# ylongqi/openrec

Hardware: AMD Instinct MI355X
Metric: BPR training triplets/sec at dim=64, 1Mx1M table (higher is better)
Workload: dtype f32; 1 GPU; bpr dim=64 1000000x1000000 table, batch=65536 triplets/GPU, sgd lr=0.05, objective loss+l2_loss, exact TF duplicate semantics; parallelism=single-gpu

## Files before the change

### include/openrec_hip.h

```cpp
#ifndef OPENREC_HIP_H
#define OPENREC_HIP_H

#include <stdint.h>

#ifdef __cplusplus
extern "C" {
#endif

typedef struct orx_ctx orx_ctx;
typedef struct orx_table orx_table;
typedef struct orx_opt orx_opt;

enum orx_status {
    ORX_OK = 0,
    ORX_ERR_ARG = -1,
    ORX_ERR_HIP = -2,
    ORX_ERR_OOM = -3,
    ORX_ERR_INDEX = -4,
    ORX_ERR_STATE = -5
};

enum orx_opt_kind { ORX_SGD = 0, ORX_ADAGRAD = 1, ORX_ADAM = 2, ORX_MOMENTUM = 3 };

enum orx_pair_model { ORX_BPR = 0, ORX_UCML = 1 };
// ... 262 lines not shown
int orx_prof_get(orx_ctx* ctx, int kid, double* total_ms, int64_t* launches);
int orx_ctx_stat(orx_ctx* ctx, int what, int64_t* out);
int orx_copy_bandwidth(orx_ctx* ctx, int64_t bytes, int32_t reps, double* gbps_out);

int orx_gemm16_plan(int32_t num_cu, int32_t M, int32_t N, int32_t K, int64_t lda, int64_t ldb, int32_t* nt_out, int32_t* tn_out);
int orx_gemm16_group_query(int32_t num_cu, int32_t B, int32_t in, int32_t out, int64_t ldx, int64_t lddz, int64_t ldw, int32_t nt_cols,
                           int32_t* plan_out);
int orx_gemm16_nt(orx_ctx* ctx, const void* A16, int64_t lda, const void* B16, int64_t ldb, float* C, int64_t ldc, void* C16, int64_t ldc16,
                  const float* bias, int32_t M, int32_t N, int32_t K, int act, const float* actY, const void* actY16, int64_t ldy, int act_y,
                  float* colparts, int32_t* P_out, void* mask_out, const void* mask_in);
int orx_gemm16_tn(orx_ctx* ctx, const void* A16, int64_t lda, const void* B16, int64_t ldb, float* C, int64_t ldc, float* slab,
                  int32_t M, int32_t N, int32_t K, float out_scale);
int orx_gemm16_group(orx_ctx* ctx, const void* X16, int64_t ldx, const void* dZ16, int64_t lddz, float* gW, int64_t ldgw, float* slab,
                     int32_t in, int32_t out, int32_t B, float out_scale, const void* W16, int64_t ldw, float* C, int64_t ldc,
                     void* C16, int64_t ldc16, const float* actY, const void* actY16, int64_t ldy, int act_y, float* colparts,
                     int32_t* P_out, const void* mask_in, int32_t nt_cols);
int orx_head16_fwd(orx_ctx* ctx, const void* X16, int64_t ldx, const void* w16, const float* bias, int act, float* pred, int32_t B, int32_t K);
int32_t orx_head16_bwd_blocks(orx_ctx* ctx, int32_t B);
int orx_head16_bwd(orx_ctx* ctx, const void* X16, int64_t ldx, const void* w16, const float* dy, const float* pred, int act, int act_below,
                   float* gW_parts, float* gb_parts, void* dZ16, int64_t ld16, float* dZ32, int64_t ld32, float* gb_below_parts,
                   int32_t B, int32_t K, int32_t* P_out);
int orx_cast16(orx_ctx* ctx, const float* src, int64_t lds, void* dst16, int64_t ld16, int32_t M, int32_t N);

int orx_plan_geometry(int64_t NU, int64_t NI, int64_t nU, int64_t nP, int64_t nN, int32_t* out);
int orx_plan_dump(orx_ctx* ctx, const int32_t* uid, const int32_t* pid, const int32_t* nid, const float* label, int64_t K, int64_t B,
                  int64_t NU, int64_t NI, int32_t D, const int32_t* opts, void* const* out, int64_t* info);

#ifdef __cplusplus
}
#endif
#endif
```

### openrec_amd/_ffi.py

```python
from __future__ import annotations

import ctypes
import os
from ctypes import POINTER, c_char_p, c_double, c_float, c_int, c_int32, c_int64, c_size_t, c_uint64, c_void_p

HERE = os.path.dirname(os.path.abspath(__file__))
LIB_PATH = os.environ.get("ORX_LIB_PATH") or os.path.join(HERE, "_lib", "libopenrec_hip.so")

ORX_OK, ORX_ERR_ARG, ORX_ERR_HIP, ORX_ERR_OOM, ORX_ERR_INDEX, ORX_ERR_STATE = 0, -1, -2, -3, -4, -5
ORX_SGD, ORX_ADAGRAD, ORX_ADAM, ORX_MOMENTUM = 0, 1, 2, 3
ORX_BPR, ORX_UCML = 0, 1
ORX_GMF, ORX_WRMF = 0, 1
ORX_IDS_DEVICE, ORX_HOGWILD, ORX_NO_L2, ORX_CENSOR, ORX_POINT_SIGMOID, ORX_OUT_DEVICE = 1, 2, 4, 8, 16, 32
ORX_TRAIN_USER, ORX_TRAIN_ITEM, ORX_TRAIN_BIAS = 1, 2, 4
ORX_SHARD_OVERLAP, ORX_SHARD_NO_DEDUP, ORX_SHARD_DEDUP, ORX_COMM_ID_BYTES = 0x100, 0x200, 0x400, 128
ORX_DLRM_INTERACT_ITSELF, ORX_DLRM_SIGMOID_BOT, ORX_DLRM_SIGMOID_TOP, ORX_DLRM_LOSS_BCE, ORX_DLRM_REFERENCE_COMPAT = 1, 2, 4, 8, 16
ORX_DLRM_FP16_MLP = 32
ORX_DLRM_NO_EMB = 64
ORX_K_DEDUP, ORX_K_FUSED, ORX_K_REDUCE, ORX_K_SWEEP, ORX_K_CENSOR, ORX_K_POINT, ORX_K_DUPAPPLY, ORX_K_GEMM, ORX_K_NUM = 0, 1, 2, 3, 4, 5, 6, 7, 8
KERNEL_NAMES = {ORX_K_DEDUP: "dedup", ORX_K_FUSED: "fused", ORX_K_REDUCE: "loss_reduce", ORX_K_SWEEP: "adam_sweep",
                ORX_K_CENSOR: "censor", ORX_K_POINT: "pointwise", ORX_K_DUPAPPLY: "dup_apply", ORX_K_GEMM: "gemm"}

_p = c_void_p
_pp = POINTER(c_void_p)
# ... 102 lines not shown
    "orx_shard_grads_sgd": (c_int, [_p, c_int, _p, _p, _fp, _ip, _ip, _p, _p, _p, _ip, _fp, _p, c_int64, c_int64, c_int64, c_float, c_int, _fp, _ip, _fp, _p]),
    "orx_shard_request_dedup_steps": (c_int, [_p, _ip, c_int64, c_int64, c_int32, c_int32, c_int64, _ip, _ip, _ip, _p, _p, _p, _ip, _ip]),
    "orx_prof_enable": (c_int, [_p, c_int]),
    "orx_prof_reset": (c_int, [_p]),
    "orx_prof_get": (c_int, [_p, c_int, POINTER(c_double), POINTER(c_int64)]),
    "orx_ctx_stat": (c_int, [_p, c_int, POINTER(c_int64)]),
    "orx_copy_bandwidth": (c_int, [_p, c_int64, c_int32, POINTER(c_double)]),
    "orx_mlp_forward": (c_int, [_p, c_int32, POINTER(_p), POINTER(_p), POINTER(c_int32), _p, c_int64, c_int32, c_int, _p]),
    "orx_interact_forward": (c_int, [_p, _p, c_int64, c_int32, c_int32, c_int, c_int, c_int, _p]),
    "orx_gemm16_plan": (c_int, [c_int32, c_int32, c_int32, c_int32, c_int64, c_int64, POINTER(c_int32), POINTER(c_int32)]),
    "orx_gemm16_group_query": (c_int, [c_int32, c_int32, c_int32, c_int32, c_int64, c_int64, c_int64, c_int32, POINTER(c_int32)]),
    "orx_gemm16_nt": (c_int, [_p, _p, c_int64, _p, c_int64, _fp, c_int64, _p, c_int64, _fp, c_int32, c_int32, c_int32, c_int,
                              _fp, _p, c_int64, c_int, _fp, POINTER(c_int32), _p, _p]),
    "orx_gemm16_tn": (c_int, [_p, _p, c_int64, _p, c_int64, _fp, c_int64, _fp, c_int32, c_int32, c_int32, c_float]),
    "orx_gemm16_group": (c_int, [_p, _p, c_int64, _p, c_int64, _fp, c_int64, _fp, c_int32, c_int32, c_int32, c_float, _p, c_int64, _fp, c_int64,
                                 _p, c_int64, _fp, _p, c_int64, c_int, _fp, POINTER(c_int32), _p, c_int32]),
    "orx_head16_fwd": (c_int, [_p, _p, c_int64, _p, _fp, c_int, _fp, c_int32, c_int32]),
    "orx_head16_bwd_blocks": (c_int32, [_p, c_int32]),
    "orx_head16_bwd": (c_int, [_p, _p, c_int64, _p, _fp, _fp, c_int, c_int, _fp, _fp, _p, c_int64, _fp, c_int64, _fp, c_int32, c_int32, POINTER(c_int32)]),
    "orx_cast16": (c_int, [_p, _fp, c_int64, _p, c_int64, c_int32, c_int32]),
    "orx_plan_geometry": (c_int, [c_int64, c_int64, c_int64, c_int64, c_int64, POINTER(c_int32)]),
    "orx_plan_dump": (c_int, [_p, _ip, _ip, _ip, _fp, c_int64, c_int64, c_int64, c_int64, c_int32, POINTER(c_int32), POINTER(c_void_p),
                              POINTER(c_int64)]),
}

_lib = None


class OrxError(RuntimeError):
    def __init__(self, code, msg):
        super().__init__(f"[orx {code}] {msg}")
        self.code = code


def load():
    global _lib
    if _lib is not None:
        return _lib
    if not os.path.exists(LIB_PATH):
        raise ImportError(
            f"{LIB_PATH} is missing: build it with `python -m openrec_amd.build` "
            "(hipcc, gfx950).  openrec_amd has no CPU fallback.")
    try:
        import torch
    except ImportError:
        pass
# ... 21 lines not shown
```

### openrec_amd/csrc/api_plan.hip

```cpp
#include "orx_internal.h"

#include <cstring>
#include <vector>

#define CHECK(call)                                                                    \
    do {                                                                               \
        int _rc = (call);                                                              \
        if (_rc != ORX_OK) return _rc;                                                 \
    } while (0)

extern "C" int orx_plan_geometry(int64_t NU, int64_t NI, int64_t nU, int64_t nP, int64_t nN, int32_t* out) {
    ORX_ARG(out && NU > 0 && NI > 0 && nU >= 0 && nP >= 0 && nN >= 0, "orx_plan_geometry: bad argument");
    DedupArgs d;
    memset(&d, 0, sizeof(d));
    d.nU = nU; d.nP = nP; d.nN = nN; d.NU = NU; d.NI = NI;
    orx_plan_geometry_query(d, out);
    out[14] = (int32_t)orx_dedup_range_rows(); out[15] = orx_dedup_buckets(NU);
    return ORX_OK;
}

namespace {
struct DevBuf {
    void* p = nullptr;
    ~DevBuf() { if (p) (void)hipFree(p); }
    int put(const void* src, size_t bytes, hipStream_t st) {
        ORX_HIP(hipMalloc(&p, bytes < 16 ? 16 : bytes));
        ORX_HIP(hipMemcpyAsync(p, src, bytes, hipMemcpyHostToDevice, st));
        return ORX_OK;
    }
};
template <class T>
int fetch(std::vector<T>* h, const T* dev, size_t n, hipStream_t st) {
    h->resize(n);
    if (n) ORX_HIP(hipMemcpyAsync(h->data(), dev, n * sizeof(T), hipMemcpyDeviceToHost, st));
    return ORX_OK;
}
}

extern "C" int orx_plan_dump(orx_ctx* c, const int32_t* uid, const int32_t* pid, const int32_t* nid, const float* label, int64_t K, int64_t B,
                             int64_t NU, int64_t NI, int32_t D, const int32_t* opts, void* const* out, int64_t* info) {
// ... 116 lines not shown
```

### openrec_amd/csrc/kernels_plan.hip

```cpp
#include "orx_internal.h"

#include "orx_device.h"

#include <cstring>
#include <vector>
#include <algorithm>

constexpr int PL_THREADS = 256;
constexpr int PL_REFS = 8;
constexpr int PL_CHUNK = PL_THREADS * PL_REFS;
constexpr int PL_LCNT = 1024;

struct PlanArgs {
    DedupArgs d;
    int shift;
    int nru, nri;
    int lgu, lgi;
    int* bcnt;
    int2* list;
    int64_t nref;
    unsigned int* dupbits;
    int min_late;
    int s_first;
    unsigned long long* tstamp;
};
#define PL_STAMP(i) do { if (a.tstamp != nullptr && threadIdx.x == 0) a.tstamp[((size_t)blockIdx.y * gridDim.x + blockIdx.x) * 8 + (i)] = wall_clock64(); } while (0)

__device__ __forceinline__ bool plan_ref(const PlanArgs& a, int64_t s, int64_t j, int& id, bool& is_user, int& pos) {
    const DedupArgs& d = a.d;
    if (j < d.nU) { id = d.uid[s * d.id_stride + j]; is_user = true; pos = (int)j; }
    else if (j < d.nU + d.nP) { id = d.pid[s * d.id_stride + (j - d.nU)]; is_user = false; pos = (int)(d.role_stride ? d.role_stride + (j - d.nU) : j); }
    else { id = d.nid[s * d.id_stride + (j - d.nU - d.nP)]; is_user = false; pos = (int)(d.role_stride ? 2 * d.role_stride + (j - d.nU - d.nP) : j); }
    return id_ok(id, is_user ? d.NU : d.NI);
}

__device__ __forceinline__ int32_t* plan_idword(const DedupArgs& d, int64_t s, int pos) {
    if (d.pair_tpw > 1) {
        const int Bp = (int)d.role_stride;
        const int slot = (pos >= Bp ? 1 : 0) + (pos >= 2 * Bp ? 1 : 0);
        return reinterpret_cast<int32_t*>(d.ids4 + s * d.pair_stride + (pos - slot * Bp)) + slot;
    }
    return d.ids_out + s * d.flag_stride + pos;
}

__device__ __forceinline__ void pl_lds_barrier() { asm volatile("s_waitcnt lgkmcnt(0)\n\ts_barrier" ::: "memory"); }

template <int T = PL_THREADS>
__device__ __forceinline__ int plan_scan_excl(int v, int* wave_tot, int& total) {
    const int lane = threadIdx.x & 63, wave = threadIdx.x >> 6;
    int incl = v;
#pragma unroll
    for (int o = 1; o < 64; o <<= 1) { const int t = __shfl_up(incl, o); if (lane >= o) incl += t; }
    if (lane == 63) wave_tot[wave] = incl;
    pl_lds_barrier();
    int before = 0, all = 0;
#pragma unroll
    for (int k = 0; k < T / 64; ++k) { const int t = wave_tot[k]; if (k < wave) before += t; all += t; }
    pl_lds_barrier();
    total = all;
    return before + incl - v;
}

template <bool SCATTER>
__global__ __launch_bounds__(PL_THREADS) void plan_part_kernel(PlanArgs a) {
    extern __shared__ int pl_hist[];
    const int nb = a.nru + a.nri;
    const int64_t s = blockIdx.y;
    int* hist = pl_hist;
    int* base = pl_hist + nb;
    for (int i = threadIdx.x; i < nb; i += PL_THREADS) hist[i] = 0;
    __syncthreads();
    const int64_t j0 = (int64_t)blockIdx.x * PL_CHUNK + threadIdx.x;
    int bk[PL_REFS], rk[PL_REFS], idv[PL_REFS], posv[PL_REFS];
#pragma unroll
    for (int k = 0; k < PL_REFS; ++k) {
        const int64_t j = j0 + (int64_t)k * PL_THREADS;
        bk[k] = -1;
        if (j < a.nref) {
            int id, pos; bool is_user;
            const bool ok = plan_ref(a, s, j, id, is_user, pos);
            if (ok) {
                bk[k] = is_user ? (id & (a.nru - 1)) : a.nru + (id & (a.nri - 1));
                idv[k] = id; posv[k] = pos;
            }
            if (SCATTER) {
                if (a.d.pair_tpw > 1) {
                    if (j < a.d.pair_stride) {
                        const int p = a.d.pid[s * a.d.id_stride + j];
                        const int n = a.d.label ? __float_as_int(a.d.label[s * a.d.id_stride + j]) : a.d.nid[s * a.d.id_stride + j];
                        const bool okp = id_ok(p, a.d.NI), okn = a.d.label ? true : id_ok(n, a.d.NI);
                        a.d.ids4[s * a.d.pair_stride + j] = make_int4(ok ? id : 0x7fffffff, okp ? p : 0x7fffffff, okn ? n : 0x7fffffff, (int)((uint32_t)j << 10));
                        if (!(ok & okp & okn)) {
                            const int poison = (int)(ORX_PARTNER_POISON | ((uint32_t)a.d.pair_gen << 24));
                            a.d.partner[s * a.d.pair_stride + j] = make_int4(poison, poison, poison, 0);
                        }
                    }
                } else {
                    a.d.ids_out[s * a.d.flag_stride + pos] = ok ? id : 0x7fffffff;
                }
            }
        }
    }
#pragma unroll
    for (int k = 0; k < PL_REFS; ++k) if (bk[k] >= 0) rk[k] = atomicAdd(&hist[bk[k]], 1);
    __syncthreads();
    int* cnt = a.bcnt + s * (3 * nb + 1);
    if (!SCATTER) {
        if (blockIdx.x == 0 && threadIdx.x < 8) a.d.alloc[8 * s + threadIdx.x] = 0;
        if (blockIdx.x == 0 && threadIdx.x == 8) a.d.dcount[s] = 0;
        for (int i = threadIdx.x; i < nb; i += PL_THREADS) { const int c = hist[i]; if (c) atomicAdd(cnt + i, c); }
        return;
    }
    __shared__ int wave_tot[PL_THREADS / 64];
    int* off = pl_hist + 2 * nb;
    for (int i = threadIdx.x; i < nb; i += PL_THREADS) off[i] = cnt[i];
    __syncthreads();
    {
        const int per = (nb + PL_THREADS - 1) / PL_THREADS;
        const int i0 = threadIdx.x * per;
        int mine = 0;
        for (int i = i0; i < i0 + per && i < nb; ++i) mine += off[i];
        int total;
        int run = plan_scan_excl(mine, wave_tot, total);
        for (int i = i0; i < i0 + per && i < nb; ++i) { const int c = off[i]; off[i] = run; run += c; }
        if (threadIdx.x == 0) off[nb] = total;
    }
    __syncthreads();
    if (blockIdx.x == 0) for (int i = threadIdx.x; i <= nb; i += PL_THREADS) cnt[2 * nb + i] = off[i];
    int* cur = cnt + nb;
    for (int i = threadIdx.x; i < nb; i += PL_THREADS) { const int c = hist[i]; if (c) base[i] = off[i] + atomicAdd(cur + i, c); }
    __syncthreads();
    int2* list = a.list + s * a.nref;
#pragma unroll
    for (int k = 0; k < PL_REFS; ++k) if (bk[k] >= 0) list[base[bk[k]] + rk[k]] = make_int2(idv[k], posv[k]);
}

__device__ __forceinline__ int pl_cnt(const int* p) { return __hip_atomic_load(p, __ATOMIC_RELAXED, __HIP_MEMORY_SCOPE_AGENT); }
__device__ __forceinline__ unsigned int pl_peek(const unsigned int* p) { return *reinterpret_cast<const volatile unsigned int*>(p); }

constexpr int PL_UN = 8;
template <int T, class F>
__device__ __forceinline__ void pl_for_each(const int2* ent, int n, F f) {
    for (int i0 = threadIdx.x; i0 < n; i0 += PL_UN * T) {
        int2 e[PL_UN];
#pragma unroll
        for (int k = 0; k < PL_UN; ++k) { const int i = i0 + k * T; if (i < n) e[k] = ent[i]; }
#pragma unroll
        for (int k = 0; k < PL_UN; ++k) { const int i = i0 + k * T; if (i < n) f(i, e[k]); }
    }
}

__device__ __forceinline__ int pl_rank(int* cnt, int dn) {
    const int lane = threadIdx.x & 63;
    int rank = -1;
    for (int round = 0; round < 4; ++round) {
        const unsigned long long todo = __ballot(rank < 0);
        if (!todo) break;
        const int ld = __shfl(dn, __ffsll((long long)todo) - 1);
        const bool mine = rank < 0 && dn == ld;
        const unsigned long long grp = __ballot(mine);
        const int gsz = __popcll(grp);
        if (gsz < 4) break;
        const int first = __ffsll((long long)grp) - 1;
        int base = 0;
        if (lane == first) base = atomicAdd(cnt + ld, gsz);
        base = __shfl(base, first);
        if (mine) rank = base + __popcll(grp & ((1ull << lane) - 1ull));
    }
    if (rank < 0) rank = atomicAdd(cnt + dn, 1);
    return rank;
}

constexpr int PL_PAIR_CAP = 512;

template <int T>
__global__ __launch_bounds__(T) void plan_range_kernel(PlanArgs a) {
    extern __shared__ __attribute__((aligned(16))) unsigned int pl_lds[];
    const DedupArgs& d = a.d;
    const int W = (1 << a.shift) >> 5;
    unsigned int* seen = pl_lds;
    unsigned int* dup = pl_lds + W;
    unsigned int* tri = pl_lds + 2 * W;
    unsigned short* prefix16 = reinterpret_cast<unsigned short*>(pl_lds + 3 * W);
    int* lcnt = reinterpret_cast<int*>(pl_lds + 3 * W + (W + 1) / 2);
    unsigned short* dprefix16 = reinterpret_cast<unsigned short*>(seen);
    int* pairpos = reinterpret_cast<int*>(lcnt + PL_LCNT);
    __shared__ int wave_tot[T / 64];
    __shared__ int sh_late, sh_dense, sh_seg, list_cnt, list_base;
    const int nb = a.nru + a.nri;
    const int b = blockIdx.x;
    const int64_t s = blockIdx.y;
    const bool is_user = b < a.nru;
    const int lg = is_user ? a.lgu : a.lgi;
    const int bl = is_user ? b : b - a.nru;
    const int* cnt = a.bcnt + s * (3 * nb + 1) + 2 * nb;
    PL_STAMP(0);
    if (b == 0) for (int i = threadIdx.x; i < 2 * nb; i += T) a.bcnt[s * (3 * nb + 1) + i] = 0;
    const int lo = cnt[b], n = cnt[b + 1] - lo;
    int2* ent = a.list + s * a.nref + lo;
    unsigned int* dupout = a.dupbits ? a.dupbits + ((size_t)s * nb + b) * W : nullptr;
    if (threadIdx.x == 0 && n > 8192) atomicMax(d.alloc + 8 * s + 6, n);
    if (n == 0) {
        if (dupout) for (int w = threadIdx.x; w < W; w += T) dupout[w] = 0u;
        return;
    }
    int2* refinfo = d.refinfo ? d.refinfo + s * d.flag_stride : nullptr;
    const bool small = n <= PL_UN * T;
    int2 er[PL_UN];
    if (small) {
// ... 42 lines not shown
    int off = 0;
    if (mine) off = atomicAdd(&list_cnt, mine);
    pl_lds_barrier();
    int list_base_r = 0;
    if (threadIdx.x == 0 && list_cnt) {
        list_base_r = atomicAdd(d.dcount + s, list_cnt);
        atomicAdd(d.alloc + 8 * s + 5, list_cnt);
    }
    const bool want_plan = sh_late >= (a.min_late < 0 ? (n / 512 > 64 ? n / 512 : 64) : a.min_late);
    const bool plan = refinfo != nullptr && want_plan;
    if (want_plan && refinfo == nullptr && threadIdx.x == 0) atomicAdd(d.alloc + 8 * s + 1, sh_late);
    int ntri = 0, dense0 = 0;
    int* segstart = nullptr;
    if (plan) {
        segstart = d.segstart + s * d.tri_stride;
        const int per = (W + T - 1) / T;
        const int w0 = threadIdx.x * per;
        int mine3 = 0;
        for (int w = w0; w < w0 + per && w < W; ++w) mine3 += __popc(tri[w]);
        int pre = plan_scan_excl<T>(mine3, wave_tot, ntri);
        if (ntri > 65535) ntri = 0;
        if (ntri) {
            if (threadIdx.x == 0) sh_dense = atomicAdd(d.alloc + 8 * s, ntri);
            for (int w = w0; w < w0 + per && w < W; ++w) { prefix16[w] = (unsigned short)pre; pre += __popc(tri[w]); }
            __syncthreads();
            dense0 = sh_dense;
            if (ntri > PL_LCNT) lcnt = d.tricnt + s * d.tri_stride + dense0;
            for (int i = threadIdx.x; i < ntri; i += T) lcnt[i] = 0;
            __syncthreads();
        }
    }
    int ndup2 = 0;
    const bool pairing = d.pair_tpw > 1 && W <= 4096;
    if (pairing) {
        const int per = (W + T - 1) / T;
        const int w0 = threadIdx.x * per;
        int mine2 = 0;
        for (int w = w0; w < w0 + per && w < W; ++w) mine2 += __popc(dup[w] & ~tri[w]);
        int pre = plan_scan_excl<T>(mine2, wave_tot, ndup2);
        if (ndup2 > PL_PAIR_CAP) ndup2 = 0;
        if (ndup2) {
            for (int w = w0; w < w0 + per && w < W; ++w) { dprefix16[w] = (unsigned short)pre; pre += __popc(dup[w] & ~tri[w]); }
            for (int i = threadIdx.x; i < 2 * ndup2; i += T) pairpos[i] = -1;
            pl_lds_barrier();
        }
    }
    PL_STAMP(3);
    auto pass2 = [&](int2 e) {
        const int l = e.x >> lg;
        const int pos = e.y & 0x3fffffff;
        const unsigned int dw = dup[l >> 5];
        const unsigned int dd = (dw >> (l & 31)) & 1u;
        if (dd) {
            uint32_t v = (uint32_t)e.x | (1u << 31);
            const unsigned int tw = tri[l >> 5];
            const unsigned int t3 = (tw >> (l & 31)) & 1u;
            if (ndup2 && !t3) {
                const int dn2 = (int)dprefix16[l >> 5] + __popc(dw & ~tw & ((1u << (l & 31)) - 1u));
                pairpos[2 * dn2 + (int)(((uint32_t)e.y >> 30) & 1u)] = pos;
                return;
            }
            v |= (t3 ? 2u : ((uint32_t)e.y >> 30)) << 29;
            if (t3 && ntri) {
                const int dn = (int)prefix16[l >> 5] + __popc(tw & ((1u << (l & 31)) - 1u));
                refinfo[pos] = make_int2(dense0 + dn, pl_rank(lcnt, dn));
            } else if (t3 && refinfo != nullptr) {
                refinfo[pos] = make_int2(-1, 0);
            }
            *plan_idword(d, s, pos) = (int32_t)v;
        }
    };
    if (small) {
#pragma unroll
        for (int k = 0; k < PL_UN; ++k) { const int i = threadIdx.x + k * T; if (i < n) pass2(er[k]); }
    } else {
        pl_for_each<T>(ent, n, [&](int, int2 e) { pass2(e); });
    }
    PL_STAMP(4);
    if (ndup2) {
        pl_lds_barrier();
        int* partner = reinterpret_cast<int*>(d.partner + s * d.pair_stride);
        const int Bp = (int)d.role_stride;
        for (int k = threadIdx.x; k < ndup2; k += T) {
            const int posA = pairpos[2 * k], posB = pairpos[2 * k + 1];
            const int sa = (posA >= Bp ? 1 : 0) + (posA >= 2 * Bp ? 1 : 0), sb = (posB >= Bp ? 1 : 0) + (posB >= 2 * Bp ? 1 : 0);
            const int tag = d.pair_gen << 24;
            partner[4 * (posA - sa * Bp) + sa] = posB | tag;
// ... 22 lines not shown
    PL_STAMP(7);
    if (mine) {
        int64_t e = s * d.list_stride + list_base + off;
        const uint32_t tag = is_user ? 0u : 0x80000000u;
        for (int w = threadIdx.x; w < W; w += T) {
            unsigned int m = dup[w];
            const unsigned int m0 = m;
            const unsigned int tw = tri[w];
            while (m) {
                const int bpos = __ffs(m) - 1;
                m &= m - 1;
                if (ndup2 && !((tw >> bpos) & 1u)) {
                    const int dn2 = (int)dprefix16[w] + __popc(m0 & ~tw & ((1u << bpos) - 1u));
                    reinterpret_cast<int2*>(d.pslot)[e] = make_int2(pairpos[2 * dn2], pairpos[2 * dn2 + 1]);
                    if (d.dcnt != nullptr) { d.dseg[e] = 0; d.dcnt[e] = 0; }
                    ++e;
                    continue;
                }
                if (d.pair_tpw > 1) reinterpret_cast<int2*>(d.pslot)[e] = make_int2(-1, -1);
                d.dlist[e] = (uint32_t)((((int64_t)w * 32 + bpos) << lg) | bl) | tag;
                if (d.dcnt != nullptr) {
                    int c = 0, sg = 0;
                    if (ntri && ((tw >> bpos) & 1u)) {
                        const int dn = (int)prefix16[w] + __popc(tw & ((1u << bpos) - 1u));
                        c = pl_cnt(lcnt + dn);
                        sg = __hip_atomic_load(segstart + dense0 + dn, __ATOMIC_RELAXED, __HIP_MEMORY_SCOPE_AGENT);
                        if (c > ORX_SEG_DIRECT) {
                            int4* items = d.items + s * d.item_stride;
                            int src = sg, len = c, level = 0;
                            do {
                                const int pieces = (len + ORX_PIECE - 1) / ORX_PIECE;
                                const int b0 = d.tree_off[level] + atomicAdd(d.alloc + 8 * s + 2 + level, pieces);
                                for (int k = 0; k < pieces; ++k) {
                                    const int rem = len - k * ORX_PIECE;
                                    items[b0 + k] = make_int4(src + k * ORX_PIECE, rem < ORX_PIECE ? rem : ORX_PIECE, b0 + k, 0);
                                }
                                src = b0; len = pieces; ++level;
                            } while (len > ORX_SEG_DIRECT && level < 3);
                            sg = src; c = -len;
                        }
                    }
                    d.dseg[e] = sg; d.dcnt[e] = c;
                }
                ++e;
            }
        }
    }
// ... 92 lines not shown
        }
    }
    __shared__ int sh_np;
    if (threadIdx.x == 0) sh_np = 0;
    __syncthreads();
    if (npair) atomicAdd(&sh_np, npair);
    __syncthreads();
    if (threadIdx.x == 0 && sh_np) atomicAdd(d.alloc + 8 * s + 7, sh_np);
}

__global__ __launch_bounds__(256) void plan_swap_kernel(DedupArgs d) {
    const int64_t s = blockIdx.y;
    const int n = d.dcount[s];
    int4* rec = d.ids4 + s * d.pair_stride;
    for (int e = blockIdx.x * 256 + threadIdx.x; e < n; e += gridDim.x * 256) {
        const int2 qm = reinterpret_cast<const int2*>(d.pslot)[s * d.list_stride + e];
        if (qm.x < 0 || qm.y < 0) continue;
        const int4 a = rec[qm.x], b = rec[qm.y];
        rec[qm.x] = make_int4(b.x, b.y, b.z, a.w);
        rec[qm.y] = make_int4(a.x, a.y, a.z, b.w);
    }
}

int orx_launch_plan_swap(orx_ctx* ctx, const DedupArgs& d, int64_t kc) {
    if (d.pair_tpw < 2 || kc <= 0) return ORX_OK;
    ProfScope ps(ctx, ORX_K_DEDUP);
    ORX_LAUNCH(ctx, plan_swap_kernel, dim3((unsigned)std::max<int64_t>(4, (d.pair_stride / 4 + 255) / 256), (unsigned)kc), dim3(256), 0, d);
    ORX_HIP(hipGetLastError());
    return ORX_OK;
}

static int plan_buckets(int64_t rows, int64_t nref_t) {
    if (rows <= 0 || nref_t <= 0) return 0;
    const int cap = rows > (1LL << 27) ? 18 : 17;
    int64_t want = std::max<int64_t>((rows + (1LL << cap) - 1) >> cap, std::min<int64_t>(nref_t / 2048, rows / 64));
    static const char* env = getenv("ORX_PLAN_SHIFT");
    if (env) want = std::max<int64_t>(want, (rows + (1LL << atoi(env)) - 1) >> atoi(env));
    int n = 1;
    while (n < want && n < 8192) n *= 2;
    return n;
}
static int ilog2(int64_t n) { int l = 0; while ((1LL << l) < n) ++l; return l; }
static void plan_geometry(const DedupArgs& d, PlanArgs* a) {
    a->nref = d.nU + d.nP + d.nN;
    a->nru = plan_buckets(d.nU ? d.NU : 0, d.nU);
    a->nri = plan_buckets((d.nP + d.nN) ? d.NI : 0, d.nP + d.nN);
    a->lgu = ilog2(a->nru > 0 ? a->nru : 1); a->lgi = ilog2(a->nri > 0 ? a->nri : 1);
    const int64_t per_u = a->nru ? (d.NU + a->nru - 1) / a->nru : 1, per_i = a->nri ? (d.NI + a->nri - 1) / a->nri : 1;
    a->shift = std::max(5, ilog2(std::max(per_u, per_i)));
}

void orx_plan_geometry_query(const DedupArgs& d, int32_t out[14]) {
    PlanArgs a;
    plan_geometry(d, &a);
    out[0] = a.nru; out[1] = a.nri; out[2] = a.lgu; out[3] = a.lgi; out[4] = a.shift; out[5] = (1 << a.shift) >> 5;
    out[6] = PL_UN; out[7] = PL_LCNT; out[8] = PL_PAIR_CAP; out[9] = ORX_SEG_DIRECT; out[10] = ORX_PIECE;
    out[11] = PL_THREADS; out[12] = 1024; out[13] = PL_CHUNK;
}

static int plan_ensure(orx_ctx* c, int64_t chunk, const PlanArgs& a, bool want_dupbits) {
    const int nb = a.nru + a.nri;
    if (orx_ensure((void**)&c->d_pl_cnt, &c->d_pl_cnt_cap, (size_t)chunk * (3 * nb + 1) * sizeof(int))) return ORX_ERR_OOM;
    if (orx_ensure((void**)&c->d_pl_list, &c->d_pl_list_cap, (size_t)chunk * a.nref * sizeof(int2))) return ORX_ERR_OOM;
    const size_t words = (size_t)nb * ((1u << a.shift) >> 5);
    if (want_dupbits && orx_ensure((void**)&c->d_dupbits, &c->d_dupbits_cap, (size_t)chunk * words * sizeof(unsigned int))) return ORX_ERR_OOM;
    return ORX_OK;
}

int orx_plan_buffers(orx_ctx* c, int64_t chunk, int64_t B, int64_t NU, int64_t NI, bool want_dupbits) {
    const int64_t shapes[3][3] = {{B, B, B}, {B, B, 0}, {0, B, 0}};
    for (const auto& sh : shapes) {
        DedupArgs d;
        memset(&d, 0, sizeof(d));
        d.nU = sh[0]; d.nP = sh[1]; d.nN = sh[2]; d.NU = NU; d.NI = NI;
        PlanArgs a;
        plan_geometry(d, &a);
        const int rc = plan_ensure(c, chunk, a, want_dupbits);
        if (rc != ORX_OK) return rc;
    }
    return ORX_OK;
// ... 5 lines not shown
    a.d = d;
    plan_geometry(d, &a);
    const int nb = a.nru + a.nri;
    if (nb == 0 || a.nref == 0 || kc == 0) return ORX_OK;
    ORX_ARG(a.nref < (1LL << 30) && kc < 65536, "plan: too many references per step (%lld) or steps (%lld)", (long long)a.nref, (long long)kc);
    { const int rc = plan_ensure(ctx, step0 + kc, a, keep_dupbits); if (rc != ORX_OK) return rc; }
    const size_t words = (size_t)nb * ((1u << a.shift) >> 5);
    a.bcnt = ctx->d_pl_cnt + step0 * (3 * nb + 1); a.list = ctx->d_pl_list + step0 * a.nref;
    a.dupbits = keep_dupbits ? ctx->d_dupbits + step0 * words : nullptr;
    a.s_first = 1;
    a.tstamp = nullptr;
    static const bool timing = getenv("ORX_PLAN_TIMING") != nullptr;
    if (timing) {
        ORX_HIP(hipMalloc((void**)&a.tstamp, (size_t)nb * kc * 8 * sizeof(unsigned long long)));
        ORX_HIP(hipMemsetAsync(a.tstamp, 0, (size_t)nb * kc * 8 * sizeof(unsigned long long), ctx->stream));
    }
    const char* ml = getenv("ORX_PLAN_MIN_LATE");
    a.min_late = ml ? atoi(ml) : d.min_late;
    if (ctx->pl_cnt_clean != ctx->d_pl_cnt || ctx->pl_cnt_clean_cap != ctx->d_pl_cnt_cap || ctx->pl_cnt_nb != nb)
        ORX_HIP(hipMemsetAsync(ctx->d_pl_cnt, 0, ctx->d_pl_cnt_cap, ctx->stream));
    ctx->pl_cnt_clean = nullptr;
    struct CleanMark { orx_ctx* c; int nb; bool ok = false;
                       ~CleanMark() { if (ok) { c->pl_cnt_clean = c->d_pl_cnt; c->pl_cnt_clean_cap = c->d_pl_cnt_cap; c->pl_cnt_nb = nb; } } } clean_mark{ctx, nb};
    const dim3 gp((unsigned)((a.nref + PL_CHUNK - 1) / PL_CHUNK), (unsigned)kc);
    const size_t hist_bytes = (size_t)(3 * nb + 1) * sizeof(int);
    ORX_ONCE_PER_DEVICE(ctx, ORX_HIP(hipFuncSetAttribute((const void*)plan_part_kernel<false>, hipFuncAttributeMaxDynamicSharedMemorySize, 128 * 1024)));
    ORX_ONCE_PER_DEVICE(ctx, ORX_HIP(hipFuncSetAttribute((const void*)plan_part_kernel<true>, hipFuncAttributeMaxDynamicSharedMemorySize, 128 * 1024)));
    ORX_ONCE_PER_DEVICE(ctx, ORX_HIP(hipFuncSetAttribute((const void*)plan_range_kernel<256>, hipFuncAttributeMaxDynamicSharedMemorySize, 140 * 1024)));
    ORX_ONCE_PER_DEVICE(ctx, ORX_HIP(hipFuncSetAttribute((const void*)plan_range_kernel<1024>, hipFuncAttributeMaxDynamicSharedMemorySize, 140 * 1024)));
    ORX_LAUNCH(ctx, (plan_part_kernel<false>), gp, dim3(PL_THREADS), hist_bytes, a);
    ORX_LAUNCH(ctx, (plan_part_kernel<true>), gp, dim3(PL_THREADS), hist_bytes, a);
    const int W = (1 << a.shift) >> 5;
    const size_t lds = (size_t)(3 * W + (W + 1) / 2) * 4 + (size_t)PL_LCNT * 4 +
                       (d.pair_tpw > 1 && W <= 4096 ? (size_t)2 * PL_PAIR_CAP * 4 : 0);
    if (ctx->plan_big) ORX_LAUNCH(ctx, plan_range_kernel<1024>, dim3((unsigned)nb, (unsigned)kc), dim3(1024), lds, a);
    else ORX_LAUNCH(ctx, plan_range_kernel<256>, dim3((unsigned)nb, (unsigned)kc), dim3(256), lds, a);
    if (d.pair_tpw > 1) ORX_LAUNCH(ctx, plan_pair_kernel, dim3((unsigned)std::max<int64_t>(4, (d.pair_stride / 4 + 255) / 256), (unsigned)kc), dim3(256), 0, a);
    ORX_HIP(hipGetLastError());
    clean_mark.ok = true;
    if (a.tstamp != nullptr) {
        ORX_HIP(hipStreamSynchronize(ctx->stream));
        std::vector<unsigned long long> h((size_t)nb * kc * 8);
        ORX_HIP(hipMemcpy(h.data(), a.tstamp, h.size() * sizeof(unsigned long long), hipMemcpyDeviceToHost));
        ORX_HIP(hipFree(a.tstamp));
        double sum[8] = {0}; unsigned long long t_min = ~0ull, t_max = 0; size_t live = 0;
        for (size_t w = 0; w < (size_t)nb * kc; ++w) {
            const unsigned long long* t = &h[w * 8];
            if (t[7] == 0) continue;
            ++live; t_min = std::min(t_min, t[0]); t_max = std::max(t_max, t[7]);
            for (int i = 1; i < 8; ++i) sum[i] += (double)(t[i] - t[i - 1]);
        }
        fprintf(stderr, "[orx plan timing] K=%lld, %zu workgroups, span %.1f us; mean us per phase: zero+cnt %.2f | pass1 %.2f | staging+prefix %.2f | pass2 %.2f | "
                "pairing %.2f | dupbits %.2f | list alloc %.2f\n", (long long)kc, live, (double)(t_max - t_min) * 0.01,
                sum[1] / live * 0.01, sum[2] / live * 0.01, sum[3] / live * 0.01, sum[4] / live * 0.01, sum[5] / live * 0.01, sum[6] / live * 0.01, sum[7] / live * 0.01);
    }
    return ORX_OK;
}

int orx_launch_plan_urgent(orx_ctx* ctx, const DedupArgs& d, int64_t kc, int64_t step0) {
    ProfScope ps(ctx, ORX_K_DEDUP);
    const int first = step0 > 0 ? 0 : 1;
    if (kc - first < 1) return ORX_OK;
    PlanArgs a;
    a.d = d;
    plan_geometry(d, &a);
    const int nb = a.nru + a.nri;
    const size_t words = (size_t)nb * ((1u << a.shift) >> 5);
    a.bcnt = ctx->d_pl_cnt + step0 * (3 * nb + 1); a.list = ctx->d_pl_list + step0 * a.nref; a.dupbits = ctx->d_dupbits + step0 * words; a.min_late = -1;
    a.s_first = first;
    a.tstamp = nullptr;
    const int W = (1 << a.shift) >> 5;
    if (ctx->plan_big) ORX_LAUNCH(ctx, plan_urgent_kernel<1024>, dim3((unsigned)(a.nru + a.nri), (unsigned)(kc - first)), dim3(1024), (size_t)W * 4, a);
    else ORX_LAUNCH(ctx, plan_urgent_kernel<256>, dim3((unsigned)(a.nru + a.nri), (unsigned)(kc - first)), dim3(256), (size_t)W * 4, a);
    ORX_HIP(hipGetLastError());
    return ORX_OK;
}
```

### openrec_amd/csrc/orx_internal.h

```cpp
#pragma once
#include <hip/hip_runtime.h>
#include <hip/hip_ext.h>

#include <cstdarg>
#include <functional>
#include <cstdint>
#include <cstdio>
#include <map>
#include <string>
#include <vector>

#include "../../include/openrec_hip.h"

void orx_set_error(const char* fmt, ...);

#define ORX_HIP(expr)                                                                  \
    do {                                                                               \
        hipError_t _e = (expr);                                                        \
        if (_e != hipSuccess) {                                                        \
            orx_set_error("%s failed: %s (%s:%d)", #expr, hipGetErrorString(_e),       \
                          __FILE__, __LINE__);                                         \
            return _e == hipErrorOutOfMemory ? ORX_ERR_OOM : ORX_ERR_HIP;              \
        }                                                                              \
    } while (0)
// ... 354 lines not shown
int orx_launch_hot_reduce(orx_ctx* ctx, const PairArgs& a, int level);

struct PairPlan { int nw; int64_t chunk; int64_t list_stride; int64_t Bp; int64_t item_stride; int tree_off[3];
                  int min_late = -1;
                  int pair_tpw = 0;
                  int64_t cap = 0; };
struct ExactChunk { bool hot = false, use_stage = false, dense_dups = false; int tree_levels = 0;
                    bool quiet = false; };
bool orx_pairing_wanted(int mode, bool role_bits, int optkind, int dim, int64_t B, int fb);
int orx_pairing_buffers(orx_ctx* c, int64_t B, int dim, PairPlan* plan);
int orx_exact_buffers(orx_ctx* c, orx_table* U, orx_table* V, int64_t K, int64_t B, int mode, bool role_bits,
                      bool inline_apply, bool staging, int nb_total, int nw, PairPlan* plan);
int orx_exact_plan_chunk(orx_ctx* c, orx_table* U, orx_table* V, const int32_t* uid, const int32_t* pid, const int32_t* nid, int64_t ds,
                         int64_t nU, int64_t nP, int64_t nN, int64_t kc, int64_t B, bool role_bits, bool inline_apply, bool staging,
                         const PairPlan& plan, ExactChunk* out, const std::function<int()>* while_waiting = nullptr);
int orx_exact_plan_issue(orx_ctx* c, orx_table* U, orx_table* V, const int32_t* uid, const int32_t* pid, const int32_t* nid, int64_t ds,
                         int64_t nU, int64_t nP, int64_t nN, int64_t kc, int64_t B, bool inline_apply, bool staging,
                         const PairPlan& plan, int64_t i0, hipEvent_t counters, const std::function<int()>* after_readback = nullptr);
int orx_exact_plan_finish(orx_ctx* c, int64_t kc, int64_t B, bool inline_apply, bool staging, int64_t i0, hipEvent_t counters, ExactChunk* out, bool pairing_on = false);
void orx_plan_dedup_args(orx_ctx* c, orx_table* U, orx_table* V, const int32_t* uid, const int32_t* pid, const int32_t* nid, int64_t ds,
                         int64_t nU, int64_t nP, int64_t nN, int64_t B, bool role_bits, bool inline_apply, bool staging,
                         const PairPlan& plan, int64_t i0, DedupArgs* out);
void orx_plan_geometry_query(const DedupArgs& d, int32_t out[14]);
void orx_exact_step_views(orx_ctx* c, const PairPlan& plan, int64_t i, int64_t B, int D, bool use_stage, PairArgs* a);
int orx_launch_rows_planned(orx_ctx* ctx, int optkind, const RowsArgs& a);
struct RowsPlan { PairPlan plan; ExactChunk ck; int64_t n = 0; bool ready = false; };
int orx_apply_rows_plan(orx_ctx* ctx, orx_table* t, const int32_t* ids, int64_t K, int64_t n, int64_t id_stride, RowsPlan* out);
int orx_apply_rows_planned_step(orx_ctx* ctx, orx_opt* opt, orx_table* t, orx_table* bias, const RowsPlan& rp, int64_t i,
                                const int32_t* ids, const float* grads, int64_t g_stride);
int orx_launch_dup_apply(orx_ctx* ctx, int optkind, const PairArgs& a);
bool orx_launch_tail(orx_ctx* ctx, int optkind, const PairArgs& a, const ReduceArgs& r, int64_t K, int* rc);
int orx_launch_urgent(orx_ctx* ctx, const DedupArgs& a, int64_t K);
bool orx_plan_v2(bool role_bits);
int orx_plan_buffers(orx_ctx* c, int64_t chunk, int64_t B, int64_t NU, int64_t NI, bool want_dupbits);
int orx_launch_plan(orx_ctx* ctx, const DedupArgs& d, int64_t kc, bool keep_dupbits, int64_t step0 = 0);
int orx_launch_plan_urgent(orx_ctx* ctx, const DedupArgs& d, int64_t kc, int64_t step0 = 0);
int orx_launch_plan_swap(orx_ctx* ctx, const DedupArgs& d, int64_t kc);
int orx_fused_tpw(int D);
int orx_fused_can_inline_apply(int D);
int orx_dedup_words(void);
int orx_launch_loss_reduce(orx_ctx* ctx, const ReduceArgs& a, int64_t K);
int orx_fused_nwaves(int D, int64_t B);
int orx_dedup_buckets(int64_t rows);
int64_t orx_dedup_range_rows();

enum { MODE_EXACT = 0,
// ... 276 lines not shown
```

Baseline: 1.042 billion triplets/s.

## Shrink plan-kernel LDS and register footprint to raise occupancy

The range kernel's shared memory is repacked: the prefix table is stored at half resolution and recomputed with an extra popcount, and it shares one pool with the seen bitmap, cutting dynamic LDS per block. The partition kernel no longer keeps per-reference positions in registers; it recomputes them on demand, and it gains a min-blocks launch bound. It also switches to a lighter LDS barrier and moves the ids_out write into the first, non-scatter pass. A new API reports per-kernel grid, LDS and occupancy so launch shapes can be inspected. The intent is more resident workgroups per CU during dedup planning, at the cost of slightly more ALU work and the risk that forced launch bounds cause register spills.

After: 979.5 million triplets/s. 0.94x the previous value.

```diff
diff --git a/include/openrec_hip.h b/include/openrec_hip.h
--- a/include/openrec_hip.h
+++ b/include/openrec_hip.h
@@ -308,6 +308,7 @@
                    int32_t B, int32_t K, int32_t* P_out);
 int orx_cast16(orx_ctx* ctx, const float* src, int64_t lds, void* dst16, int64_t ld16, int32_t M, int32_t N);
 
+int orx_plan_launch_shape(orx_ctx* ctx, int64_t NU, int64_t NI, int64_t B, int64_t K, int32_t pairing, int32_t* out, int32_t* num_cu);
 int orx_plan_geometry(int64_t NU, int64_t NI, int64_t nU, int64_t nP, int64_t nN, int32_t* out);
 int orx_plan_dump(orx_ctx* ctx, const int32_t* uid, const int32_t* pid, const int32_t* nid, const float* label, int64_t K, int64_t B,
                   int64_t NU, int64_t NI, int32_t D, const int32_t* opts, void* const* out, int64_t* info);
diff --git a/openrec_amd/_ffi.py b/openrec_amd/_ffi.py
--- a/openrec_amd/_ffi.py
+++ b/openrec_amd/_ffi.py
@@ -148,6 +148,7 @@
     "orx_plan_geometry": (c_int, [c_int64, c_int64, c_int64, c_int64, c_int64, POINTER(c_int32)]),
     "orx_plan_dump": (c_int, [_p, _ip, _ip, _ip, _fp, c_int64, c_int64, c_int64, c_int64, c_int32, POINTER(c_int32), POINTER(c_void_p),
                               POINTER(c_int64)]),
+    "orx_plan_launch_shape": (c_int, [_p, c_int64, c_int64, c_int64, c_int64, c_int32, POINTER(c_int32), POINTER(c_int32)]),
 }
 
 _lib = None
diff --git a/openrec_amd/csrc/api_plan.hip b/openrec_amd/csrc/api_plan.hip
--- a/openrec_amd/csrc/api_plan.hip
+++ b/openrec_amd/csrc/api_plan.hip
@@ -16,6 +16,18 @@
     d.nU = nU; d.nP = nP; d.nN = nN; d.NU = NU; d.NI = NI;
     orx_plan_geometry_query(d, out);
     out[14] = (int32_t)orx_dedup_range_rows(); out[15] = orx_dedup_buckets(NU);
+    return ORX_OK;
+}
+
+extern "C" int orx_plan_launch_shape(orx_ctx* c, int64_t NU, int64_t NI, int64_t B, int64_t K, int32_t pairing, int32_t* out, int32_t* num_cu) {
+    ORX_ARG(c && out && num_cu && NU > 0 && NI > 0 && B > 0 && K > 0 && K < 65536, "orx_plan_launch_shape: bad argument");
+    ORX_HIP(hipSetDevice(c->device));
+    DedupArgs d;
+    memset(&d, 0, sizeof(d));
+    d.nU = d.nP = d.nN = B; d.NU = NU; d.NI = NI;
+    if (pairing) { d.pair_tpw = 2; d.pair_stride = B; }
+    CHECK(orx_plan_launch_shape_query(c, d, K, reinterpret_cast<int32_t(*)[4]>(out)));
+    *num_cu = c->num_cu;
     return ORX_OK;
 }
 
diff --git a/openrec_amd/csrc/kernels_plan.hip b/openrec_amd/csrc/kernels_plan.hip
--- a/openrec_amd/csrc/kernels_plan.hip
+++ b/openrec_amd/csrc/kernels_plan.hip
@@ -26,11 +26,16 @@
 };
 #define PL_STAMP(i) do { if (a.tstamp != nullptr && threadIdx.x == 0) a.tstamp[((size_t)blockIdx.y * gridDim.x + blockIdx.x) * 8 + (i)] = wall_clock64(); } while (0)
 
-__device__ __forceinline__ bool plan_ref(const PlanArgs& a, int64_t s, int64_t j, int& id, bool& is_user, int& pos) {
+__device__ __forceinline__ int plan_pos(const DedupArgs& d, int64_t j) {
+    if (j < d.nU || !d.role_stride) return (int)j;
+    return (int)(j < d.nU + d.nP ? d.role_stride + (j - d.nU) : 2 * d.role_stride + (j - d.nU - d.nP));
+}
+
+__device__ __forceinline__ bool plan_ref(const PlanArgs& a, int64_t s, int64_t j, int& id, bool& is_user) {
     const DedupArgs& d = a.d;
-    if (j < d.nU) { id = d.uid[s * d.id_stride + j]; is_user = true; pos = (int)j; }
-    else if (j < d.nU + d.nP) { id = d.pid[s * d.id_stride + (j - d.nU)]; is_user = false; pos = (int)(d.role_stride ? d.role_stride + (j - d.nU) : j); }
-    else { id = d.nid[s * d.id_stride + (j - d.nU - d.nP)]; is_user = false; pos = (int)(d.role_stride ? 2 * d.role_stride + (j - d.nU - d.nP) : j); }
+    if (j < d.nU) { id = d.uid[s * d.id_stride + j]; is_user = true; }
+    else if (j < d.nU + d.nP) { id = d.pid[s * d.id_stride + (j - d.nU)]; is_user = false; }
+    else { id = d.nid[s * d.id_stride + (j - d.nU - d.nP)]; is_user = false; }
     return id_ok(id, is_user ? d.NU : d.NI);
 }
 
@@ -62,28 +67,28 @@
 }
 
 template <bool SCATTER>
-__global__ __launch_bounds__(PL_THREADS) void plan_part_kernel(PlanArgs a) {
+__global__ __launch_bounds__(PL_THREADS, 8) void plan_part_kernel(PlanArgs a) {
     extern __shared__ int pl_hist[];
     const int nb = a.nru + a.nri;
     const int64_t s = blockIdx.y;
     int* hist = pl_hist;
     int* base = pl_hist + nb;
     for (int i = threadIdx.x; i < nb; i += PL_THREADS) hist[i] = 0;
-    __syncthreads();
+    pl_lds_barrier();
     const int64_t j0 = (int64_t)blockIdx.x * PL_CHUNK + threadIdx.x;
-    int bk[PL_REFS], rk[PL_REFS], idv[PL_REFS], posv[PL_REFS];
+    int bk[PL_REFS], rk[PL_REFS], idv[PL_REFS];
 #pragma unroll
     for (int k = 0; k < PL_REFS; ++k) {
         const int64_t j = j0 + (int64_t)k * PL_THREADS;
         bk[k] = -1;
         if (j < a.nref) {
-            int id, pos; bool is_user;
-            const bool ok = plan_ref(a, s, j, id, is_user, pos);
+            int id; bool is_user;
+            const bool ok = plan_ref(a, s, j, id, is_user);
             if (ok) {
                 bk[k] = is_user ? (id & (a.nru - 1)) : a.nru + (id & (a.nri - 1));
-                idv[k] = id; posv[k] = pos;
+                idv[k] = id;
             }
-            if (SCATTER) {
+            if (!SCATTER) {
                 if (a.d.pair_tpw > 1) {
                     if (j < a.d.pair_stride) {
                         const int p = a.d.pid[s * a.d.id_stride + j];
@@ -96,14 +101,14 @@
                         }
                     }
                 } else {
-                    a.d.ids_out[s * a.d.flag_stride + pos] = ok ? id : 0x7fffffff;
+                    a.d.ids_out[s * a.d.flag_stride + plan_pos(a.d, j)] = ok ? id : 0x7fffffff;
                 }
             }
         }
     }
 #pragma unroll
     for (int k = 0; k < PL_REFS; ++k) if (bk[k] >= 0) rk[k] = atomicAdd(&hist[bk[k]], 1);
-    __syncthreads();
+    pl_lds_barrier();
     int* cnt = a.bcnt + s * (3 * nb + 1);
     if (!SCATTER) {
         if (blockIdx.x == 0 && threadIdx.x < 8) a.d.alloc[8 * s + threadIdx.x] = 0;
@@ -114,7 +119,7 @@
     __shared__ int wave_tot[PL_THREADS / 64];
     int* off = pl_hist + 2 * nb;
     for (int i = threadIdx.x; i < nb; i += PL_THREADS) off[i] = cnt[i];
-    __syncthreads();
+    pl_lds_barrier();
     {
         const int per = (nb + PL_THREADS - 1) / PL_THREADS;
         const int i0 = threadIdx.x * per;
@@ -125,14 +130,15 @@
         for (int i = i0; i < i0 + per && i < nb; ++i) { const int c = off[i]; off[i] = run; run += c; }
         if (threadIdx.x == 0) off[nb] = total;
     }
-    __syncthreads();
+    pl_lds_barrier();
     if (blockIdx.x == 0) for (int i = threadIdx.x; i <= nb; i += PL_THREADS) cnt[2 * nb + i] = off[i];
     int* cur = cnt + nb;
     for (int i = threadIdx.x; i < nb; i += PL_THREADS) { const int c = hist[i]; if (c) base[i] = off[i] + atomicAdd(cur + i, c); }
-    __syncthreads();
+    pl_lds_barrier();
     int2* list = a.list + s * a.nref;
 #pragma unroll
-    for (int k = 0; k < PL_REFS; ++k) if (bk[k] >= 0) list[base[bk[k]] + rk[k]] = make_int2(idv[k], posv[k]);
+    for (int k = 0; k < PL_REFS; ++k)
+        if (bk[k] >= 0) list[base[bk[k]] + rk[k]] = make_int2(idv[k], plan_pos(a.d, j0 + (int64_t)k * PL_THREADS));
 }
 
 __device__ __forceinline__ int pl_cnt(const int* p) { return __hip_atomic_load(p, __ATOMIC_RELAXED, __HIP_MEMORY_SCOPE_AGENT); }
@@ -173,18 +179,28 @@
 
 constexpr int PL_PAIR_CAP = 512;
 
+__host__ __device__ constexpr bool pl_pair_tables(int pair_tpw, int W) { return pair_tpw > 1 && W <= 4096; }
+__host__ __device__ constexpr int pl_dprefix_words(int W) { return (W + 1) / 2; }
+__host__ __device__ constexpr int pl_prefix_words(int W) { return ((W + 1) / 2 + 1) / 2; }
+__host__ __device__ constexpr int pl_pool_words(int W, bool pair_tables) {
+    return pl_dprefix_words(W) + pl_prefix_words(W) + PL_LCNT + (pair_tables ? 2 * PL_PAIR_CAP : 0);
+}
+__host__ __device__ constexpr int pl_range_lds_words(int W, bool pair_tables) {
+    return 2 * W + (pl_pool_words(W, pair_tables) > W ? pl_pool_words(W, pair_tables) : W);
+}
+
 template <int T>
-__global__ __launch_bounds__(T) void plan_range_kernel(PlanArgs a) {
+__global__ __launch_bounds__(T, T == 256 ? 8 : 4) void plan_range_kernel(PlanArgs a) {
     extern __shared__ __attribute__((aligned(16))) unsigned int pl_lds[];
     const DedupArgs& d = a.d;
     const int W = (1 << a.shift) >> 5;
-    unsigned int* seen = pl_lds;
-    unsigned int* dup = pl_lds + W;
-    unsigned int* tri = pl_lds + 2 * W;
-    unsigned short* prefix16 = reinterpret_cast<unsigned short*>(pl_lds + 3 * W);
-    int* lcnt = reinterpret_cast<int*>(pl_lds + 3 * W + (W + 1) / 2);
+    unsigned int* dup = pl_lds;
+    unsigned int* tri = pl_lds + W;
+    unsigned int* seen = pl_lds + 2 * W;
     unsigned short* dprefix16 = reinterpret_cast<unsigned short*>(seen);
-    int* pairpos = reinterpret_cast<int*>(lcnt + PL_LCNT);
+    unsigned short* prefix16 = reinterpret_cast<unsigned short*>(seen + pl_dprefix_words(W));
+    int* lcnt = reinterpret_cast<int*>(seen + pl_dprefix_words(W) + pl_prefix_words(W));
+    int* pairpos = lcnt + PL_LCNT;
     __shared__ int wave_tot[T / 64];
     __shared__ int sh_late, sh_dense, sh_seg, list_cnt, list_base;
     const int nb = a.nru + a.nri;
@@ -273,7 +289,7 @@
         if (ntri > 65535) ntri = 0;
         if (ntri) {
             if (threadIdx.x == 0) sh_dense = atomicAdd(d.alloc + 8 * s, ntri);
-            for (int w = w0; w < w0 + per && w < W; ++w) { prefix16[w] = (unsigned short)pre; pre += __popc(tri[w]); }
+            for (int w = w0; w < w0 + per && w < W; ++w) { if (!(w & 1)) prefix16[w >> 1] = (unsigned short)pre; pre += __popc(tri[w]); }
             __syncthreads();
             dense0 = sh_dense;
             if (ntri > PL_LCNT) lcnt = d.tricnt + s * d.tri_stride + dense0;
@@ -282,7 +298,7 @@
         }
     }
     int ndup2 = 0;
-    const bool pairing = d.pair_tpw > 1 && W <= 4096;
+    const bool pairing = pl_pair_tables(d.pair_tpw, W);
     if (pairing) {
         const int per = (W + T - 1) / T;
         const int w0 = threadIdx.x * per;
@@ -297,6 +313,9 @@
         }
     }
     PL_STAMP(3);
+    auto pl_tri_dense = [&](int w, unsigned int tw, int bit) {
+        return (int)prefix16[w >> 1] + ((w & 1) ? __popc(tri[w - 1]) : 0) + __popc(tw & ((1u << bit) - 1u));
+    };
     auto pass2 = [&](int2 e) {
         const int l = e.x >> lg;
         const int pos = e.y & 0x3fffffff;
@@ -313,7 +332,7 @@
             }
             v |= (t3 ? 2u : ((uint32_t)e.y >> 30)) << 29;
             if (t3 && ntri) {
-                const int dn = (int)prefix16[l >> 5] + __popc(tw & ((1u << (l & 31)) - 1u));
+                const int dn = pl_tri_dense(l >> 5, tw, l & 31);
                 refinfo[pos] = make_int2(dense0 + dn, pl_rank(lcnt, dn));
             } else if (t3 && refinfo != nullptr) {
                 refinfo[pos] = make_int2(-1, 0);
@@ -382,7 +401,7 @@
                 if (d.dcnt != nullptr) {
                     int c = 0, sg = 0;
                     if (ntri && ((tw >> bpos) & 1u)) {
-                        const int dn = (int)prefix16[w] + __popc(tw & ((1u << bpos) - 1u));
+                        const int dn = pl_tri_dense(w, tw, bpos);
                         c = pl_cnt(lcnt + dn);
                         sg = __hip_atomic_load(segstart + dense0 + dn, __ATOMIC_RELAXED, __HIP_MEMORY_SCOPE_AGENT);
                         if (c > ORX_SEG_DIRECT) {
@@ -521,10 +540,12 @@
     }
 }
 
+static dim3 plan_list_grid(const DedupArgs& d, int64_t kc) { return dim3((unsigned)std::max<int64_t>(4, (d.pair_stride / 4 + 255) / 256), (unsigned)kc); }
+
 int orx_launch_plan_swap(orx_ctx* ctx, const DedupArgs& d, int64_t kc) {
     if (d.pair_tpw < 2 || kc <= 0) return ORX_OK;
     ProfScope ps(ctx, ORX_K_DEDUP);
-    ORX_LAUNCH(ctx, plan_swap_kernel, dim3((unsigned)std::max<int64_t>(4, (d.pair_stride / 4 + 255) / 256), (unsigned)kc), dim3(256), 0, d);
+    ORX_LAUNCH(ctx, plan_swap_kernel, plan_list_grid(d, kc), dim3(256), 0, d);
     ORX_HIP(hipGetLastError());
     return ORX_OK;
 }
@@ -555,6 +576,44 @@
     out[0] = a.nru; out[1] = a.nri; out[2] = a.lgu; out[3] = a.lgi; out[4] = a.shift; out[5] = (1 << a.shift) >> 5;
     out[6] = PL_UN; out[7] = PL_LCNT; out[8] = PL_PAIR_CAP; out[9] = ORX_SEG_DIRECT; out[10] = ORX_PIECE;
     out[11] = PL_THREADS; out[12] = 1024; out[13] = PL_CHUNK;
+}
+
+static dim3 plan_part_grid(const PlanArgs& a, int64_t kc) { return dim3((unsigned)((a.nref + PL_CHUNK - 1) / PL_CHUNK), (unsigned)kc); }
+static size_t plan_part_lds(const PlanArgs& a) { return (size_t)(3 * (a.nru + a.nri) + 1) * sizeof(int); }
+static dim3 plan_range_grid(const PlanArgs& a, int64_t kc) { return dim3((unsigned)(a.nru + a.nri), (unsigned)kc); }
+static size_t plan_range_lds(const PlanArgs& a, const DedupArgs& d) {
+    const int W = (1 << a.shift) >> 5;
+    return (size_t)pl_range_lds_words(W, pl_pair_tables(d.pair_tpw, W)) * 4;
+}
+static size_t plan_urgent_lds(const PlanArgs& a) { return (size_t)((1 << a.shift) >> 5) * 4; }
+static int plan_func_attributes(orx_ctx* ctx) {
+    ORX_ONCE_PER_DEVICE(ctx, ORX_HIP(hipFuncSetAttribute((const void*)plan_part_kernel<false>, hipFuncAttributeMaxDynamicSharedMemorySize, 128 * 1024)));
+    ORX_ONCE_PER_DEVICE(ctx, ORX_HIP(hipFuncSetAttribute((const void*)plan_part_kernel<true>, hipFuncAttributeMaxDynamicSharedMemorySize, 128 * 1024)));
+    ORX_ONCE_PER_DEVICE(ctx, ORX_HIP(hipFuncSetAttribute((const void*)plan_range_kernel<256>, hipFuncAttributeMaxDynamicSharedMemorySize, 140 * 1024)));
+    ORX_ONCE_PER_DEVICE(ctx, ORX_HIP(hipFuncSetAttribute((const void*)plan_range_kernel<1024>, hipFuncAttributeMaxDynamicSharedMemorySize, 140 * 1024)));
+    return ORX_OK;
+}
+
+int orx_plan_launch_shape_query(orx_ctx* ctx, const DedupArgs& d, int64_t kc, int32_t out[6][4]) {
+    PlanArgs a;
+    plan_geometry(d, &a);
+    { const int rc = plan_func_attributes(ctx); if (rc != ORX_OK) return rc; }
+    const bool pairing = d.pair_tpw > 1;
+    const dim3 gp = plan_part_grid(a, kc), gr = plan_range_grid(a, kc), gl = plan_list_grid(d, kc);
+    struct { const void* f; int64_t wgs; int threads; size_t lds; } k[6] = {
+        {(const void*)plan_part_kernel<false>, (int64_t)gp.x * gp.y, PL_THREADS, plan_part_lds(a)},
+        {(const void*)plan_part_kernel<true>, (int64_t)gp.x * gp.y, PL_THREADS, plan_part_lds(a)},
+        {(const void*)plan_range_kernel<256>, (int64_t)gr.x * gr.y, 256, plan_range_lds(a, d)},
+        {(const void*)plan_pair_kernel, pairing ? (int64_t)gl.x * gl.y : 0, 256, 0},
+        {(const void*)plan_urgent_kernel<256>, (int64_t)gr.x * std::max<int64_t>(0, kc - 1), 256, plan_urgent_lds(a)},
+        {(const void*)plan_swap_kernel, pairing ? (int64_t)gl.x * gl.y : 0, 256, 0},
+    };
+    for (int i = 0; i < 6; ++i) {
+        int per_cu = 0;
+        ORX_HIP(hipOccupancyMaxActiveBlocksPerMultiprocessor(&per_cu, k[i].f, k[i].threads, k[i].lds));
+        out[i][0] = (int32_t)k[i].wgs; out[i][1] = k[i].threads; out[i][2] = (int32_t)k[i].lds; out[i][3] = per_cu;
+    }
+    return ORX_OK;
 }
 
 static int plan_ensure(orx_ctx* c, int64_t chunk, const PlanArgs& a, bool want_dupbits) {
@@ -606,20 +665,12 @@
     ctx->pl_cnt_clean = nullptr;
     struct CleanMark { orx_ctx* c; int nb; bool ok = false;
                        ~CleanMark() { if (ok) { c->pl_cnt_clean = c->d_pl_cnt; c->pl_cnt_clean_cap = c->d_pl_cnt_cap; c->pl_cnt_nb = nb; } } } clean_mark{ctx, nb};
-    const dim3 gp((unsigned)((a.nref + PL_CHUNK - 1) / PL_CHUNK), (unsigned)kc);
-    const size_t hist_bytes = (size_t)(3 * nb + 1) * sizeof(int);
-    ORX_ONCE_PER_DEVICE(ctx, ORX_HIP(hipFuncSetAttribute((const void*)plan_part_kernel<false>, hipFuncAttributeMaxDynamicSharedMemorySize, 128 * 1024)));
-    ORX_ONCE_PER_DEVICE(ctx, ORX_HIP(hipFuncSetAttribute((const void*)plan_part_kernel<true>, hipFuncAttributeMaxDynamicSharedMemorySize, 128 * 1024)));
-    ORX_ONCE_PER_DEVICE(ctx, ORX_HIP(hipFuncSetAttribute((const void*)plan_range_kernel<256>, hipFuncAttributeMaxDynamicSharedMemorySize, 140 * 1024)));
-    ORX_ONCE_PER_DEVICE(ctx, ORX_HIP(hipFuncSetAttribute((const void*)plan_range_kernel<1024>, hipFuncAttributeMaxDynamicSharedMemorySize, 140 * 1024)));
-    ORX_LAUNCH(ctx, (plan_part_kernel<false>), gp, dim3(PL_THREADS), hist_bytes, a);
-    ORX_LAUNCH(ctx, (plan_part_kernel<true>), gp, dim3(PL_THREADS), hist_bytes, a);
-    const int W = (1 << a.shift) >> 5;
-    const size_t lds = (size_t)(3 * W + (W + 1) / 2) * 4 + (size_t)PL_LCNT * 4 +
-                       (d.pair_tpw > 1 && W <= 4096 ? (size_t)2 * PL_PAIR_CAP * 4 : 0);
-    if (ctx->plan_big) ORX_LAUNCH(ctx, plan_range_kernel<1024>, dim3((unsigned)nb, (unsigned)kc), dim3(1024), lds, a);
-    else ORX_LAUNCH(ctx, plan_range_kernel<256>, dim3((unsigned)nb, (unsigned)kc), dim3(256), lds, a);
-    if (d.pair_tpw > 1) ORX_LAUNCH(ctx, plan_pair_kernel, dim3((unsigned)std::max<int64_t>(4, (d.pair_stride / 4 + 255) / 256), (unsigned)kc), dim3(256), 0, a);
+    { const int rc = plan_func_attributes(ctx); if (rc != ORX_OK) return rc; }
+    ORX_LAUNCH(ctx, (plan_part_kernel<false>), plan_part_grid(a, kc), dim3(PL_THREADS), plan_part_lds(a), a);
+    ORX_LAUNCH(ctx, (plan_part_kernel<true>), plan_part_grid(a, kc), dim3(PL_THREADS), plan_part_lds(a), a);
+    if (ctx->plan_big) ORX_LAUNCH(ctx, plan_range_kernel<1024>, plan_range_grid(a, kc), dim3(1024), plan_range_lds(a, d), a);
+    else ORX_LAUNCH(ctx, plan_range_kernel<256>, plan_range_grid(a, kc), dim3(256), plan_range_lds(a, d), a);
+    if (d.pair_tpw > 1) ORX_LAUNCH(ctx, plan_pair_kernel, plan_list_grid(d, kc), dim3(256), 0, a);
     ORX_HIP(hipGetLastError());
     clean_mark.ok = true;
     if (a.tstamp != nullptr) {
@@ -653,9 +704,8 @@
     a.bcnt = ctx->d_pl_cnt + step0 * (3 * nb + 1); a.list = ctx->d_pl_list + step0 * a.nref; a.dupbits = ctx->d_dupbits + step0 * words; a.min_late = -1;
     a.s_first = first;
     a.tstamp = nullptr;
-    const int W = (1 << a.shift) >> 5;
-    if (ctx->plan_big) ORX_LAUNCH(ctx, plan_urgent_kernel<1024>, dim3((unsigned)(a.nru + a.nri), (unsigned)(kc - first)), dim3(1024), (size_t)W * 4, a);
-    else ORX_LAUNCH(ctx, plan_urgent_kernel<256>, dim3((unsigned)(a.nru + a.nri), (unsigned)(kc - first)), dim3(256), (size_t)W * 4, a);
+    if (ctx->plan_big) ORX_LAUNCH(ctx, plan_urgent_kernel<1024>, plan_range_grid(a, kc - first), dim3(1024), plan_urgent_lds(a), a);
+    else ORX_LAUNCH(ctx, plan_urgent_kernel<256>, plan_range_grid(a, kc - first), dim3(256), plan_urgent_lds(a), a);
     ORX_HIP(hipGetLastError());
     return ORX_OK;
 }
diff --git a/openrec_amd/csrc/orx_internal.h b/openrec_amd/csrc/orx_internal.h
--- a/openrec_amd/csrc/orx_internal.h
+++ b/openrec_amd/csrc/orx_internal.h
@@ -400,6 +400,7 @@
                          int64_t nU, int64_t nP, int64_t nN, int64_t B, bool role_bits, bool inline_apply, bool staging,
                          const PairPlan& plan, int64_t i0, DedupArgs* out);
 void orx_plan_geometry_query(const DedupArgs& d, int32_t out[14]);
+int orx_plan_launch_shape_query(orx_ctx* ctx, const DedupArgs& d, int64_t kc, int32_t out[6][4]);
 void orx_exact_step_views(orx_ctx* c, const PairPlan& plan, int64_t i, int64_t B, int D, bool use_stage, PairArgs* a);
 int orx_launch_rows_planned(orx_ctx* ctx, int optkind, const RowsArgs& a);
 struct RowsPlan { PairPlan plan; ExactChunk ck; int64_t n = 0; bool ready = false; };
```
